# yugabyte/yugabyte-db

Measured on NVIDIA H100. Metric: compaction GB/s (input bytes merged), higher is better.
Workload: dtype u8

## Files before the change

yugabyte-db_b200/csrc/encode_kernels.cuh:

```cuda
#pragma once

namespace ybgpu {

constexpr int SEG = 4096;
constexpr int GROUP_SEGS = 64;

struct EncView {
  const RunView* runs;
  const Desc* kept;
  const ValueRewrite* rewrites;
  uint32_t* nr;
  uint16_t* shared;
  int16_t* D;
  unsigned long long* P;
  unsigned long long* QQ;
  uint32_t* next;
  uint32_t* exit1;
  uint32_t n;
  uint32_t ri;
  uint32_t ri_shift;
  uint32_t block_size;
  uint32_t deviation;
  uint32_t guess;
  int key_encoding;
// ... 130 lines not shown
  for (uint32_t base = 0; base < n; base += 1024) {
    uint32_t i = base + threadIdx.x;
    unsigned long long v = i < n ? a[i] : 0, x = v;
    for (int o = 1; o < 32; o <<= 1) { unsigned long long y = __shfl_up_sync(0xffffffffu, x, o); if (lane >= o) x += y; }
    if (lane == 31) ws[wid] = x;
    __syncthreads();
    if (wid == 0) {
      unsigned long long w = ws[lane];
      for (int o = 1; o < 32; o <<= 1) { unsigned long long y = __shfl_up_sync(0xffffffffu, w, o); if (lane >= o) w += y; }
      ws[lane] = w;
    }
    __syncthreads();
    if (i < n) a[i] = carry + (wid ? ws[wid - 1] : 0) + x - v;
    __syncthreads();
    if (threadIdx.x == 1023) carry += ws[31];
    __syncthreads();
  }
  if (threadIdx.x == 0 && total) *total = carry;
}
__global__ void __launch_bounds__(256) k_u64_chunk_sums(const unsigned long long* a, uint32_t n, unsigned long long* partial) {
  __shared__ unsigned long long sh;
  if (threadIdx.x == 0) sh = 0;
  __syncthreads();
  unsigned long long s = 0;
  const uint64_t base = static_cast<uint64_t>(blockIdx.x) * SCAN_CHUNK;
  for (uint32_t j = threadIdx.x; j < SCAN_CHUNK; j += 256) { const uint64_t i = base + j; if (i < n) s += a[i]; }
  for (int o = 16; o; o >>= 1) s += __shfl_xor_sync(0xffffffffu, s, o);
  if ((threadIdx.x & 31) == 0) atomicAdd(&sh, s);
  __syncthreads();
  if (threadIdx.x == 0) partial[blockIdx.x] = sh;
}
__global__ void __launch_bounds__(256) k_u64_chunk_final(unsigned long long* a, uint32_t n, const unsigned long long* partial) {
  __shared__ unsigned long long ws[8];
  const uint64_t base = static_cast<uint64_t>(blockIdx.x) * SCAN_CHUNK;
  constexpr int PER = SCAN_CHUNK / 256;
  const int lane = threadIdx.x & 31, wid = threadIdx.x >> 5;
  unsigned long long v[PER], s = 0;
  for (int j = 0; j < PER; j++) { const uint64_t i = base + threadIdx.x * PER + j; v[j] = i < n ? a[i] : 0; s += v[j]; }
  unsigned long long x = s;
  for (int o = 1; o < 32; o <<= 1) { const unsigned long long y = __shfl_up_sync(0xffffffffu, x, o); if (lane >= o) x += y; }
  if (lane == 31) ws[wid] = x;
  __syncthreads();
  unsigned long long run = partial[blockIdx.x] + x - s;
  for (int w = 0; w < wid; w++) run += ws[w];
  for (int j = 0; j < PER; j++) {
    const uint64_t i = base + threadIdx.x * PER + j;
    if (i < n) a[i] = run;
    run += v[j];
  }
}
__global__ void __launch_bounds__(256) k_p_final(const uint32_t* nr, uint32_t n, const unsigned long long* partial, unsigned long long* P) {
  __shared__ uint32_t warp_sums[32];
  const uint64_t base = static_cast<uint64_t>(blockIdx.x) * SCAN_CHUNK;
  constexpr int PER = SCAN_CHUNK / 256;
  uint32_t v[PER], s = 0;
  for (int j = 0; j < PER; j++) { uint64_t i = base + threadIdx.x * PER + j; v[j] = i < n ? nr[i] : 0; s += v[j]; }
  uint32_t off = block_exclusive_scan(s, warp_sums, nullptr);
  unsigned long long run = partial[blockIdx.x] + off;
  for (int j = 0; j < PER; j++) {
    uint64_t i = base + threadIdx.x * PER + j;
    if (i < n) P[i] = run;
    run += v[j];
    if (i + 1 == n) P[n] = run;
  }
}

constexpr int QROWS = 128;
__global__ void __launch_bounds__(256) k_qq_sums(const int16_t* D, uint32_t n, uint32_t ri, unsigned long long* partial , uint32_t nchunks) {
  const uint32_t t = blockIdx.x * blockDim.x + threadIdx.x;
  const uint32_t chunk = t / ri, col = t % ri;
  if (chunk >= nchunks) return;
  unsigned long long s = 0;
  for (int r = 0; r < QROWS; r++) {
    uint64_t i = (static_cast<uint64_t>(chunk) * QROWS + r) * ri + col;
    if (i < n) s += static_cast<unsigned long long>(static_cast<long long>(D[i]));
  }
  partial[static_cast<size_t>(col) * nchunks + chunk] = s;
}
__global__ void __launch_bounds__(256) k_qq_final(const int16_t* D, uint32_t n, uint32_t ri, const unsigned long long* partial, uint32_t nchunks, unsigned long long* QQ) {
  const uint32_t t = blockIdx.x * blockDim.x + threadIdx.x;
  const uint32_t chunk = t / ri, col = t % ri;
  if (chunk >= nchunks) return;
  unsigned long long s = partial[static_cast<size_t>(col) * nchunks + chunk];
  for (int r = 0; r < QROWS; r++) {
    uint64_t i = (static_cast<uint64_t>(chunk) * QROWS + r) * ri + col;
    if (i < n) { s += static_cast<unsigned long long>(static_cast<long long>(D[i])); QQ[i] = s; }
  }
}

__device__ __forceinline__ unsigned long long blk_cur(const EncView& E, uint32_t s, uint32_t j) {
  const uint32_t t = (j - s) >> E.ri_shift;
  return (E.P[j + 1] - E.P[s]) + (E.QQ[s + (t << E.ri_shift)] - E.QQ[s] + static_cast<unsigned long long>(static_cast<long long>(E.D[s]))) + 4ull * (t + 1) + 4ull;
}

__global__ void __launch_bounds__(256) k_next(EncView E) {
  const unsigned long long BS = E.block_size;
  const unsigned long long thresh = BS * (100 - E.deviation);
  const unsigned long long madd = *E.max_add;
  for (uint32_t s = blockIdx.x * blockDim.x + threadIdx.x; s < E.n; s += gridDim.x * blockDim.x) {
    uint32_t lo = s + 1, hi = E.n;
    if (E.deviation == 0) {
      while (lo < hi) { uint32_t mid = lo + ((hi - lo) >> 1); if (blk_cur(E, s, mid - 1) >= BS) hi = mid; else lo = mid + 1; }
      E.next[s] = lo;
      continue;
    }
    {
      uint32_t m = s + E.guess + (E.guess >> 3);
      for (int it = 0; it < 3 && lo < hi; it++) {
        if (m < lo) m = lo;
        if (m > hi) m = hi;
        const unsigned long long cur = blk_cur(E, s, m - 1);
        const unsigned long long have = cur * 100;
        const unsigned long long bpe = cur / (m - s) + 1;
        if (have > thresh) {
          hi = m;
          const unsigned long long over = (have - thresh) / 100;
          const unsigned long long back = over / bpe + 1;
          m = back >= m - s ? s + 1 : m - static_cast<uint32_t>(back);
        } else {
          lo = m < E.n ? m + 1 : E.n;
          const unsigned long long miss = (thresh - have) / 100;
          const unsigned long long fwd = miss / bpe + 1;
          m = fwd >= E.n - m ? E.n : m + static_cast<uint32_t>(fwd);
        }
      }
    }
    while (lo < hi) {
      uint32_t mid = lo + ((hi - lo) >> 1);
      if (blk_cur(E, s, mid - 1) * 100 > thresh) hi = mid; else lo = mid + 1;
    }
    uint32_t m = lo;
    if (m < E.n && BS > madd) {
      const unsigned long long lim = BS - madd;
      uint32_t a = m, b = E.n, g = m;
      for (int it = 0; it < 3 && a < b; it++) {
        if (g < a) g = a;
        if (g > b) g = b;
        const unsigned long long c = blk_cur(E, s, g - 1);
        const unsigned long long bpe = c / (g - s) + 1;
        if (c > lim) {
          b = g;
          const unsigned long long back = (c - lim) / bpe + 1;
          g = back >= g - a ? a : g - static_cast<uint32_t>(back);
        } else {
          a = g < E.n ? g + 1 : E.n;
          const unsigned long long fwd = (lim - c) / bpe + 1;
          g = fwd >= E.n - g ? E.n : g + static_cast<uint32_t>(fwd);
        }
      }
      while (a < b) {
        const uint32_t mid = a + ((b - a) >> 1);
        if (blk_cur(E, s, mid - 1) > lim) b = mid; else a = mid + 1;
      }
      m = a;
    }
    while (m < E.n) {
      const unsigned long long cur = blk_cur(E, s, m - 1);
      if (cur >= BS) break;
      const Desc d = E.kept[m];
      const unsigned long long est = cur + d.klen + d.vlen_out + ((((m - s) & (E.ri - 1)) == 0) ? 4 : 0) + 4 +
                                     varint_len(d.klen) + varint_len(d.vlen_out);
      if (est > BS && cur * 100 > thresh) break;
      m++;
    }
    E.next[s] = m;
  }
}

__global__ void __launch_bounds__(256) k_seg_exit(EncView E) {
  __shared__ uint32_t ex[SEG];
  const uint64_t b = static_cast<uint64_t>(blockIdx.x) * SEG;
  if (b >= E.n) return;
  const uint32_t e = static_cast<uint32_t>(umin64(b + SEG, E.n));
  const uint32_t cnt = e - static_cast<uint32_t>(b);
  for (uint32_t i = threadIdx.x; i < cnt; i += blockDim.x) ex[i] = E.next[b + i];
  __syncthreads();
  for (;;) {
    int changed = 0;
    for (uint32_t i = threadIdx.x; i < cnt; i += blockDim.x) {
      const uint32_t v = reinterpret_cast<volatile uint32_t*>(ex)[i];
      if (v < e) { reinterpret_cast<volatile uint32_t*>(ex)[i] = reinterpret_cast<volatile uint32_t*>(ex)[v - static_cast<uint32_t>(b)]; changed = 1; }
    }
    if (!__syncthreads_or(changed)) break;
  }
  for (uint32_t i = threadIdx.x; i < cnt; i += blockDim.x) E.exit1[b + i] = ex[i];
}

__global__ void __launch_bounds__(256) k_group_exit(EncView E, uint32_t* gexit, uint32_t ngroups) {
  const uint64_t t = blockIdx.x * static_cast<uint64_t>(blockDim.x) + threadIdx.x;
  const uint32_t g = static_cast<uint32_t>(t / SEG), q = static_cast<uint32_t>(t % SEG);
  if (g >= ngroups) return;
  const uint64_t gb = static_cast<uint64_t>(g) * SEG * GROUP_SEGS;
  const uint64_t ge = umin64(gb + static_cast<uint64_t>(SEG) * GROUP_SEGS, E.n);
  uint64_t s = gb + q;
  if (s >= E.n) { gexit[t] = E.n; return; }
  while (s < ge) s = E.exit1[s];
  gexit[t] = static_cast<uint32_t>(s);
}

__global__ void k_chain_groups(EncView E, const uint32_t* gexit, uint32_t ngroups, uint32_t* group_first) {
  if (threadIdx.x || blockIdx.x) return;
  for (uint32_t g = 0; g < ngroups; g++) group_first[g] = 0xffffffffu;
  uint64_t s = 0;
  const uint64_t GS = static_cast<uint64_t>(SEG) * GROUP_SEGS;
  while (s < E.n) {
    const uint32_t g = static_cast<uint32_t>(s / GS);
    if (group_first[g] == 0xffffffffu) group_first[g] = static_cast<uint32_t>(s);
    const uint64_t q = s - g * GS;
    if (q < SEG) s = gexit[static_cast<uint64_t>(g) * SEG + q];
    else s = E.exit1[s];
  }
}

__global__ void __launch_bounds__(128) k_group_fill(EncView E, const uint32_t* group_first, uint32_t ngroups, uint32_t* seg_first, uint32_t nsegs) {
  const uint32_t g = blockIdx.x * blockDim.x + threadIdx.x;
  if (g >= ngroups) return;
  const uint32_t s0 = static_cast<uint32_t>(g) * GROUP_SEGS, s1 = min(s0 + GROUP_SEGS, nsegs);
  for (uint32_t q = s0; q < s1; q++) seg_first[q] = 0xffffffffu;
  uint64_t s = group_first[g];
  if (s == 0xffffffffu) return;
  const uint64_t ge = umin64((static_cast<uint64_t>(g) + 1) * SEG * GROUP_SEGS, E.n);
  while (s < ge) {
    const uint32_t seg = static_cast<uint32_t>(s / SEG);
    if (seg_first[seg] == 0xffffffffu) seg_first[seg] = static_cast<uint32_t>(s);
    s = E.exit1[s];
  }
}

__global__ void __launch_bounds__(128) k_mark_starts(EncView E, const uint32_t* seg_first, uint32_t nsegs, uint8_t* is_start) {
  const uint32_t seg = blockIdx.x * blockDim.x + threadIdx.x;
  if (seg >= nsegs) return;
  uint64_t s = seg_first[seg];
  if (s == 0xffffffffu) return;
  const uint64_t e = umin64((static_cast<uint64_t>(seg) + 1) * SEG, E.n);
  while (s < e) { is_start[s] = 1; s = E.next[s]; }
}

__global__ void __launch_bounds__(256) k_start_sums(const uint8_t* is_start, uint32_t n, uint32_t* partial) {
  __shared__ uint32_t sh;
  if (threadIdx.x == 0) sh = 0;
  __syncthreads();
  uint32_t s = 0;
  const uint64_t base = static_cast<uint64_t>(blockIdx.x) * SCAN_CHUNK;
  for (uint32_t j = threadIdx.x; j < SCAN_CHUNK; j += 256) { uint64_t i = base + j; if (i < n) s += is_start[i]; }
  for (int o = 16; o; o >>= 1) s += __shfl_xor_sync(0xffffffffu, s, o);
  if ((threadIdx.x & 31) == 0) atomicAdd(&sh, s);
  __syncthreads();
  if (threadIdx.x == 0) partial[blockIdx.x] = sh;
}
__global__ void __launch_bounds__(256) k_block_first(const uint8_t* is_start, uint32_t n, const uint32_t* partial, uint32_t* block_first) {
  __shared__ uint32_t warp_sums[32];
  const uint64_t base = static_cast<uint64_t>(blockIdx.x) * SCAN_CHUNK;
  constexpr int PER = SCAN_CHUNK / 256;
  uint32_t s = 0;
  uint8_t f[PER];
  for (int j = 0; j < PER; j++) { uint64_t i = base + threadIdx.x * PER + j; f[j] = i < n ? is_start[i] : 0; s += f[j]; }
  uint32_t off = partial[blockIdx.x] + block_exclusive_scan(s, warp_sums, nullptr);
  for (int j = 0; j < PER; j++) if (f[j]) block_first[off++] = static_cast<uint32_t>(base + threadIdx.x * PER + j);
}

__global__ void __launch_bounds__(256) k_block_sizes(EncView E, const uint32_t* block_first, uint32_t nblocks, unsigned long long* block_off,
                                                     unsigned long long* max_size) {
  unsigned long long mx = 0;
  for (uint32_t b = blockIdx.x * blockDim.x + threadIdx.x; b < nblocks; b += gridDim.x * blockDim.x) {
    const uint32_t s = block_first[b], e = (b + 1 < nblocks) ? block_first[b + 1] : E.n;
    const unsigned long long sz = blk_cur(E, s, e - 1) + 5;
    block_off[b] = sz;
    mx = sz > mx ? sz : mx;
  }
  for (int o = 16; o; o >>= 1) { const unsigned long long y = __shfl_xor_sync(0xffffffffu, mx, o); mx = y > mx ? y : mx; }
  if ((threadIdx.x & 31) == 0 && mx) atomicMax(max_size, mx);
}

__device__ __forceinline__ int put_varint(uint8_t* p, uint32_t v) {
  int n = 0;
  while (v >= 128) { p[n++] = static_cast<uint8_t>(v | 128); v >>= 7; }
  p[n++] = static_cast<uint8_t>(v);
  return n;
}

__device__ uint32_t g_crc_tab[4][256];
__device__ uint32_t g_crc_x2n[32];
constexpr uint32_t CRC_XPOW_TABLE = 1u << 16;
__device__ uint32_t g_crc_xpow8[CRC_XPOW_TABLE + 1];
constexpr uint32_t CRC_STRIDE_WORDS = 256;
__device__ uint32_t g_crc_stride[4][256];
__device__ uint32_t g_crc_s32[4][256];

__global__ void k_crc_init() {
  const uint32_t i = threadIdx.x;
  uint32_t c = i;
  for (int k = 0; k < 8; k++) c = (c >> 1) ^ ((c & 1) ? 0x82F63B78u : 0u);
  g_crc_tab[0][i] = c;
  __syncthreads();
  for (int t = 1; t < 4; t++) {
    uint32_t prev = g_crc_tab[t - 1][i];
    g_crc_tab[t][i] = (prev >> 8) ^ g_crc_tab[0][prev & 0xff];
    __syncthreads();
  }
  if (i == 0) {
    auto mul = [](uint32_t a, uint32_t b) {
      uint32_t m = 1u << 31, p = 0;
      for (;;) {
        if (a & m) { p ^= b; if ((a & (m - 1)) == 0) break; }
        m >>= 1;
        b = (b & 1) ? (b >> 1) ^ 0x82F63B78u : b >> 1;
      }
      return p;
    };
// ... 1196 lines not shown
```

yugabyte-db_b200/csrc/engine.cu:

```cuda
#include "engine.h"
#include "host_sst.h"

#include <cuda_runtime.h>
#include <algorithm>
#include <cstdio>
#include <cstring>
#include <chrono>
#include <cstdlib>
#include <mutex>

namespace ybgpu {

#define CUDA_TRY(expr)                                                                      \
  do {                                                                                      \
    cudaError_t _e = (expr);                                                                \
    if (_e != cudaSuccess) {                                                                \
      return Fail(YBGPU_RUNTIME_ERROR, std::string(#expr) + ": " + cudaGetErrorString(_e)); \
    }                                                                                       \
  } while (0)

struct RunView {
  const uint8_t* data;
  const uint64_t* blk_off;
  const uint32_t* blk_size;
// ... 1271 lines not shown
    case DEV_ERR_BAD_ENTRY: return "bad entry in block";
    case DEV_ERR_COMPRESSED: return "compressed block (only kNoCompression, kSnappyCompression, kLZ4Compression and kLZ4HCCompression inputs are supported)";
    case DEV_ERR_KEY_TOO_LONG: return "key longer than the engine limit";
    case DEV_ERR_IRREGULAR_RESTARTS: return "data block restart intervals are not uniform";
    case DEV_ERR_BAD_KEY: return "cannot decode DocKey/SubDocKey components";
    case DEV_ERR_UNSUPPORTED_KEY: return "key component type not supported on the GPU path";
    case DEV_ERR_TILE_OVERFLOW: return "internal error: merge tile larger than its capacity";
    case DEV_ERR_BAD_HT: return "bad DocHybridTime at the end of a key";
    case DEV_ERR_BAD_VALUE: return "cannot decode value control fields";
    case DEV_ERR_STACK_DEPTH: return "too many subkey levels";
    case DEV_ERR_UNSUPPORTED_VALUE: return "record type needs a host callback (packed row / merge / single delete)";
    case DEV_ERR_BAD_CRC: return "block checksum mismatch";
    case DEV_ERR_COTABLE: return "cotable/colocated keys are not supported yet";
    case DEV_ERR_SHORT_KEY: return "internal key shorter than 8 bytes";
    case DEV_ERR_UNSORTED: return "input file is not sorted";
    default: return "unknown device error";
  }
}

static ybgpu_status DevErrorStatus(int e) {
  switch (e) {
    case DEV_ERR_COMPRESSED: case DEV_ERR_UNSUPPORTED_KEY: case DEV_ERR_UNSUPPORTED_VALUE:
    case DEV_ERR_TILE_OVERFLOW: case DEV_ERR_COTABLE: case DEV_ERR_KEY_TOO_LONG: case DEV_ERR_STACK_DEPTH:
    case DEV_ERR_IRREGULAR_RESTARTS:
      return YBGPU_NOT_SUPPORTED;
    default: return YBGPU_CORRUPTION;
  }
}

struct Engine::Impl {
  cudaStream_t stream = nullptr;
  bool owns_stream = false;
  uint8_t* status_host = nullptr; uint8_t* status_dev = nullptr;
  uint32_t readback_launches = 0;
  struct KvInput { const uint8_t* keys; const unsigned long long* koff; const unsigned long long* voff; uint32_t n; uint32_t max_klen; std::string last_user_key; };
  std::vector<KvInput> kv;
  std::vector<std::vector<uint32_t>> cf_oids;
  std::vector<std::vector<uint64_t>> cf_hts;
  uint8_t* staging_host = nullptr; uint8_t* staging_dev = nullptr;
  size_t upload_off = 0;
  cudaEvent_t ev0 = nullptr, ev1 = nullptr;
  cudaEvent_t phase_ev[8] = {};
  cudaEvent_t enc_ev[2] = {};
  bool enc_timed = false;
  cudaEvent_t snap_ev[4] = {};
  bool snap_timed = false;
  std::vector<void*> allocs;
  JobDev* dJ = nullptr;
  JobParams* dP = nullptr;
  RunView* dRuns = nullptr;
  std::vector<RunView> runs;
  std::vector<bool> owns_data;
  std::vector<std::vector<uint64_t>> keep_off; std::vector<std::vector<uint32_t>> keep_sz;
  uint8_t* out_keys = nullptr; uint64_t* out_koff = nullptr;
  uint8_t* out_vals = nullptr; uint64_t* out_voff = nullptr;
  uint64_t n_out = 0, out_key_bytes = 0, out_val_bytes = 0;
  JobDev hJ{};
  Desc* d_desc = nullptr; Sums3* d_partial = nullptr; ValueRewrite* d_rw = nullptr;
  uint64_t N = 0; int S = 0; uint32_t n_chunks = 0;
  bool kv_emitted = false;
  Desc* d_kept = nullptr;
  uint8_t* out_file = nullptr; uint64_t out_file_len = 0;
  uint32_t n_blocks = 0; unsigned long long* d_block_off = nullptr; uint32_t* d_block_first = nullptr;
  uint8_t* d_boundary = nullptr; uint32_t boundary_stride = 0;
  EncView enc{};
  cudaStream_t copy_stream = nullptr; cudaEvent_t copy_ev = nullptr; bool copy_pending = false;
  uint32_t n_filter_blocks = 0, filter_block_bytes = 0, filter_key_stride = 0;
  uint8_t* d_filters = nullptr; uint8_t* d_filter_keys = nullptr; uint32_t* d_filter_first = nullptr;
  BvOut* d_bv = nullptr;
};

__global__ void __launch_bounds__(256) k_records_from_kv(const uint8_t* keys, const unsigned long long* koff, const unsigned long long* voff,
                                                         const uint8_t* vals, uint32_t n, int S, uint8_t* rec, uint64_t* val_off, JobDev* J) {
  for (uint32_t i = blockIdx.x * blockDim.x + threadIdx.x; i < n; i += gridDim.x * blockDim.x) {
    const unsigned long long k0 = koff[i], k1 = koff[i + 1], v0 = voff[i], v1 = voff[i + 1];
    uint8_t* r = rec + static_cast<size_t>(i) * S;
    if (k1 < k0 + 8 || k1 - k0 - 8 > static_cast<unsigned long long>(S - 16) || v1 < v0 || v1 - v0 >= (1ull << 32)) {
      dev_fail(J, k1 < k0 + 8 ? DEV_ERR_SHORT_KEY : DEV_ERR_BAD_ENTRY, i);
      for (int b = 0; b < S; b++) r[b] = 0;
      val_off[i] = 0;
      continue;
    }
    const uint32_t ulen = static_cast<uint32_t>(k1 - k0 - 8), vlen = static_cast<uint32_t>(v1 - v0);
    const uint8_t* kp = keys + k0;
    for (int b = 0; b < S - 16; b++) r[b] = static_cast<uint32_t>(b) < ulen ? kp[b] : 0;
    uint64_t suffix = 0;
    for (int b = 7; b >= 0; b--) suffix = (suffix << 8) | kp[ulen + b];
    uint4 tr;
    tr.x = static_cast<uint32_t>(suffix); tr.y = static_cast<uint32_t>(suffix >> 32);
    tr.z = ulen | (static_cast<uint32_t>(vlen ? vals[v0] : 0) << 16);
    tr.w = vlen;
    *reinterpret_cast<uint4*>(r + S - 16) = tr;
    val_off[i] = v0;
  }
}

__global__ void k_readback(uint8_t* dst_mapped, const uint8_t* src, uint32_t n) {
  for (uint32_t i = threadIdx.x; i < n; i += blockDim.x) dst_mapped[i] = src[i];
  __threadfence_system();
}
constexpr size_t STATUS_READ_BYTES = 4096;
constexpr size_t STATUS_PAGE_BYTES = 65536;
struct StatusPage { uint8_t* host = nullptr; uint8_t* dev = nullptr; };
static std::mutex g_status_mu;
static std::vector<StatusPage> g_status_free;
static cudaError_t AcquireStatusPage(StatusPage* p) {
// ... 29 lines not shown
  if (e != cudaSuccess) { cudaFreeHost(h); return e; }
  p->host = static_cast<uint8_t*>(h); p->dev = static_cast<uint8_t*>(d);
  return cudaSuccess;
}
static void ReleaseStaging(const Staging& p) {
  if (!p.host) return;
  std::lock_guard<std::mutex> lock(g_status_mu);
  g_staging_free.push_back(p);
}
__global__ void __launch_bounds__(256) k_copy_out(uint8_t* dst_mapped, const uint8_t* src, size_t row_bytes, size_t src_pitch, size_t rows) {
  const size_t total = row_bytes * rows;
  const size_t stride = static_cast<size_t>(gridDim.x) * blockDim.x;
  if (src_pitch == row_bytes && ((reinterpret_cast<uintptr_t>(src) | reinterpret_cast<uintptr_t>(dst_mapped)) & 15) == 0) {
    const size_t nv = total >> 4;
    for (size_t i = blockIdx.x * static_cast<size_t>(blockDim.x) + threadIdx.x; i < nv; i += stride)
      reinterpret_cast<uint4*>(dst_mapped)[i] = reinterpret_cast<const uint4*>(src)[i];
    for (size_t i = (nv << 4) + blockIdx.x * static_cast<size_t>(blockDim.x) + threadIdx.x; i < total; i += stride) dst_mapped[i] = src[i];
  } else {
    for (size_t r = blockIdx.x; r < rows; r += gridDim.x)
      for (size_t c = threadIdx.x; c < row_bytes; c += blockDim.x) dst_mapped[r * row_bytes + c] = src[r * src_pitch + c];
  }
  __threadfence_system();
}

static bool ZeroCopyStatusEnabled() {
  const char* e = getenv("YBGPU_ZC_STATUS");
  return e ? atoi(e) != 0 : true;
}

Engine::Engine(const ybgpu_job_options& o) : opt_(o), impl_(new Impl) {
  if (o.largest_user_key && o.has_largest_user_key) largest_.assign(o.largest_user_key, o.largest_user_key + o.largest_user_key_len);
  if (o.key_bounds_lower_len) lower_.assign(o.key_bounds_lower, o.key_bounds_lower + o.key_bounds_lower_len);
  if (o.key_bounds_upper_len) upper_.assign(o.key_bounds_upper, o.key_bounds_upper + o.key_bounds_upper_len);
  if (o.range_lower_len) range_lower_.assign(o.range_lower, o.range_lower + o.range_lower_len);
  if (o.range_upper_len) range_upper_.assign(o.range_upper, o.range_upper + o.range_upper_len);
  opt_.range_lower = nullptr; opt_.range_upper = nullptr;
  opt_.largest_user_key = nullptr; opt_.key_bounds_lower = nullptr; opt_.key_bounds_upper = nullptr;
  memset(&stats_, 0, sizeof(stats_));
}

Engine::~Engine() {
  if (impl_) {
    cudaSetDevice(opt_.device);
    if (impl_->copy_pending) cudaStreamSynchronize(impl_->copy_stream);
    if (!ran_ && !impl_->runs.empty()) cudaStreamSynchronize(impl_->stream);
    for (void* p : impl_->allocs) cudaFreeAsync(p, impl_->stream);
    if (impl_->ev0) cudaEventDestroy(impl_->ev0);
    if (impl_->ev1) cudaEventDestroy(impl_->ev1);
    if (impl_->copy_stream) cudaStreamDestroy(impl_->copy_stream);
    if (impl_->copy_ev) cudaEventDestroy(impl_->copy_ev);
    for (auto& e : impl_->enc_ev) if (e) cudaEventDestroy(e);
    for (auto& e : impl_->snap_ev) if (e) cudaEventDestroy(e);
    for (auto& e : impl_->phase_ev) if (e) cudaEventDestroy(e);
    if (impl_->staging_host) { Staging st; st.host = impl_->staging_host; st.dev = impl_->staging_dev; ReleaseStaging(st); }
    if (impl_->status_host) {
      cudaStreamSynchronize(impl_->stream);
      StatusPage pg; pg.host = impl_->status_host; pg.dev = impl_->status_dev;
      ReleaseStatusPage(pg);
    }
    if (impl_->owns_stream && impl_->stream) cudaStreamDestroy(impl_->stream);
    delete impl_;
  }
}

ybgpu_status Engine::Fail(ybgpu_status s, const std::string& msg) { error_ = msg; return s; }

static thread_local cudaStream_t g_alloc_stream = nullptr;
template <typename T>
static cudaError_t DevAlloc(std::vector<void*>* allocs, T** out, size_t count) {
  void* p = nullptr;
  cudaError_t e = cudaMallocAsync(&p, std::max<size_t>(count * sizeof(T), 16) + 32, g_alloc_stream);
  if (e == cudaSuccess) { allocs->push_back(p); *out = reinterpret_cast<T*>(p); }
  return e;
}


static size_t CopyChunkBytes() {
  const char* e = getenv("YBGPU_COPY_CHUNK_MB");
  const long mb = e ? atol(e) : 32;
  return mb > 0 ? static_cast<size_t>(mb) << 20 : ~static_cast<size_t>(0);
}
static cudaError_t ChunkedCopyAsync(void* dst, const void* src, size_t len, cudaMemcpyKind kind, cudaStream_t stream) {
  const size_t chunk = CopyChunkBytes();
  for (size_t off = 0; off < len; off += chunk) {
    cudaError_t e = cudaMemcpyAsync(static_cast<uint8_t*>(dst) + off, static_cast<const uint8_t*>(src) + off, std::min(chunk, len - off), kind, stream);
    if (e != cudaSuccess) return e;
  }
  return cudaSuccess;
}

ybgpu_status Engine::Init() {
  int ndev = 0;
  cudaError_t e = cudaGetDeviceCount(&ndev);
  if (e != cudaSuccess || ndev == 0)
    return Fail(YBGPU_RUNTIME_ERROR, std::string("no usable CUDA device: ") + cudaGetErrorString(e) +
                                         " (this engine has no CPU fallback)");
  if (opt_.device < 0 || opt_.device >= ndev) return Fail(YBGPU_INVALID_ARGUMENT, "bad device ordinal");
  CUDA_TRY(cudaSetDevice(opt_.device));
  if (opt_.cuda_stream == YBGPU_STREAM_PRIVATE) {
    CUDA_TRY(cudaStreamCreateWithFlags(&impl_->stream, cudaStreamNonBlocking));
    impl_->owns_stream = true;
  } else {
    impl_->stream = reinterpret_cast<cudaStream_t>(opt_.cuda_stream);
  }
  g_alloc_stream = impl_->stream;
  {
    cudaMemPool_t pool;
    CUDA_TRY(cudaDeviceGetDefaultMemPool(&pool, opt_.device));
    uint64_t thr = ~0ull;
    CUDA_TRY(cudaMemPoolSetAttribute(pool, cudaMemPoolAttrReleaseThreshold, &thr));
    int off = 0;
    CUDA_TRY(cudaMemPoolSetAttribute(pool, cudaMemPoolReuseAllowInternalDependencies, &off));
  }
  if (ZeroCopyStatusEnabled()) {
    StatusPage pg;
    CUDA_TRY(AcquireStatusPage(&pg));
    impl_->status_host = pg.host; impl_->status_dev = pg.dev;
  }
  CUDA_TRY(cudaEventCreate(&impl_->ev0));
  CUDA_TRY(cudaEventCreate(&impl_->ev1));
  for (auto& e : impl_->phase_ev) CUDA_TRY(cudaEventCreate(&e));
  for (auto& e : impl_->enc_ev) CUDA_TRY(cudaEventCreate(&e));
  CUDA_TRY(DevAlloc(&impl_->allocs, &impl_->dJ, 1));
  CUDA_TRY(DevAlloc(&impl_->allocs, &impl_->dP, 1));
  CUDA_TRY(DevAlloc(&impl_->allocs, &impl_->dRuns, MAX_RUNS));
  return YBGPU_OK;
}

ybgpu_status Engine::AddInput(const uint8_t* data, uint64_t len, const ybgpu_block_handle* handles, uint64_t nh,
                              int key_encoding, uint64_t ht_filter, bool on_device) {
  if (ran_) return Fail(YBGPU_ILLEGAL_STATE, "add_input after run");
  if (impl_->runs.size() >= MAX_RUNS) return Fail(YBGPU_NOT_SUPPORTED, "too many input files");
  if (!impl_->kv.empty()) return Fail(YBGPU_NOT_SUPPORTED, "KV-stream inputs and table-file inputs cannot be mixed in one job");
  if (key_encoding != YBGPU_KEY_ENCODING_SHARED_PREFIX && key_encoding != YBGPU_KEY_ENCODING_THREE_SHARED_PARTS)
    return Fail(YBGPU_INVALID_ARGUMENT, "unknown data block key encoding");
  if (nh >= (1ull << 32)) return Fail(YBGPU_NOT_SUPPORTED, "too many data blocks in one file");
  CUDA_TRY(cudaSetDevice(opt_.device));
  g_alloc_stream = impl_->stream;
  for (uint64_t i = 0; i < nh; i++) {
    if (handles[i].offset > len || handles[i].size > len - handles[i].offset || len - handles[i].offset - handles[i].size < 5)
      return Fail(YBGPU_CORRUPTION, "block handle outside the data file");
    if (handles[i].size >= (1ull << 31)) return Fail(YBGPU_NOT_SUPPORTED, "data block too large");
  }
  RunView rv{};
  if (on_device) {
    rv.data = data;
  } else {
    uint8_t* d = nullptr;
    CUDA_TRY(DevAlloc(&impl_->allocs, &d, len + 64));
    CUDA_TRY(cudaMemsetAsync(d, 0, 16, impl_->stream));
    CUDA_TRY(ChunkedCopyAsync(d + 16, data, len, cudaMemcpyHostToDevice, impl_->stream));
    CUDA_TRY(cudaMemsetAsync(d + 16 + len, 0, 16, impl_->stream));
    rv.data = d + 16;
    stats_.h2d_bytes += len;
  }
  impl_->keep_off.emplace_back(nh); impl_->keep_sz.emplace_back(nh);
  std::vector<uint64_t>& off = impl_->keep_off.back(); std::vector<uint32_t>& sz = impl_->keep_sz.back();
  for (uint64_t i = 0; i < nh; i++) { off[i] = handles[i].offset; sz[i] = static_cast<uint32_t>(handles[i].size); }
  uint64_t* doff = nullptr; uint32_t* dsz = nullptr; uint32_t* dcnt = nullptr;
  CUDA_TRY(DevAlloc(&impl_->allocs, &doff, nh)); CUDA_TRY(DevAlloc(&impl_->allocs, &dsz, nh));
  CUDA_TRY(DevAlloc(&impl_->allocs, &dcnt, nh + 1));
  CUDA_TRY(cudaMemcpyAsync(doff, off.data(), nh * 8, cudaMemcpyHostToDevice, impl_->stream));
  CUDA_TRY(cudaMemcpyAsync(dsz, sz.data(), nh * 4, cudaMemcpyHostToDevice, impl_->stream));
  rv.blk_off = doff; rv.blk_size = dsz; rv.blk_count = dcnt; rv.nb = static_cast<uint32_t>(nh);
  rv.ht_filter = ht_filter;
  rv.key_encoding = static_cast<uint32_t>(key_encoding);
  impl_->runs.push_back(rv);
  impl_->cf_oids.emplace_back(); impl_->cf_hts.emplace_back();
  return YBGPU_OK;
}

ybgpu_status Engine::SetCotableFilters(const uint32_t* db_oids, const uint64_t* hybrid_times, uint32_t n) {
  if (ran_) return Fail(YBGPU_ILLEGAL_STATE, "set_cotable_filters after run");
  if (impl_->runs.empty()) return Fail(YBGPU_ILLEGAL_STATE, "set_cotable_filters before any input");
  if (n && (!db_oids || !hybrid_times)) return Fail(YBGPU_INVALID_ARGUMENT, "null cotable filter arrays");
  for (uint32_t i = 1; i < n; i++)
    if (db_oids[i - 1] >= db_oids[i]) return Fail(YBGPU_INVALID_ARGUMENT, "cotable filter database oids must be strictly increasing");
  impl_->cf_oids.back().assign(db_oids, db_oids + n);
  impl_->cf_hts.back().assign(hybrid_times, hybrid_times + n);
  return YBGPU_OK;
}

ybgpu_status Engine::AddInputKv(const uint8_t* keys, const uint64_t* key_offsets, const uint8_t* values, const uint64_t* value_offsets, uint64_t n) {
  Impl& I = *impl_;
  if (ran_) return Fail(YBGPU_ILLEGAL_STATE, "add_input after run");
  if (I.runs.size() >= MAX_RUNS) return Fail(YBGPU_NOT_SUPPORTED, "too many input files");
  if (I.kv.size() != I.runs.size()) return Fail(YBGPU_NOT_SUPPORTED, "KV-stream inputs and table-file inputs cannot be mixed in one job");
  if (n >= (1ull << 32)) return Fail(YBGPU_NOT_SUPPORTED, "more than 2^32 entries in one input");
  if (n && (!keys || !key_offsets || !value_offsets)) return Fail(YBGPU_INVALID_ARGUMENT, "null argument");
  CUDA_TRY(cudaSetDevice(opt_.device));
  g_alloc_stream = I.stream;
  const uint64_t kbytes = n ? key_offsets[n] : 0, vbytes = n ? value_offsets[n] : 0;
  uint32_t max_klen = 0;
  for (uint64_t i = 0; i < n; i++) {
    if (key_offsets[i + 1] < key_offsets[i] + 8 || value_offsets[i + 1] < value_offsets[i]) return Fail(YBGPU_INVALID_ARGUMENT, "bad key / value offsets");
    max_klen = std::max<uint32_t>(max_klen, static_cast<uint32_t>(std::min<uint64_t>(key_offsets[i + 1] - key_offsets[i], 0xffffffffu)));
  }
  uint8_t* dk = nullptr; uint8_t* dv = nullptr; unsigned long long* dko = nullptr; unsigned long long* dvo = nullptr; uint32_t* dcnt = nullptr;
  CUDA_TRY(DevAlloc(&I.allocs, &dk, kbytes + 16));
  CUDA_TRY(DevAlloc(&I.allocs, &dv, vbytes + 64));
  CUDA_TRY(DevAlloc(&I.allocs, &dko, n + 1)); CUDA_TRY(DevAlloc(&I.allocs, &dvo, n + 1)); CUDA_TRY(DevAlloc(&I.allocs, &dcnt, 1));
  CUDA_TRY(cudaMemsetAsync(dv, 0, 16, I.stream));
  if (kbytes) CUDA_TRY(ChunkedCopyAsync(dk, keys, kbytes, cudaMemcpyHostToDevice, I.stream));
  if (vbytes) CUDA_TRY(ChunkedCopyAsync(dv + 16, values, vbytes, cudaMemcpyHostToDevice, I.stream));
  CUDA_TRY(cudaMemsetAsync(dv + 16 + vbytes, 0, 16, I.stream));
  static const uint64_t zero_off[1] = {0};
  CUDA_TRY(ChunkedCopyAsync(dko, n ? key_offsets : zero_off, (n + 1) * 8, cudaMemcpyHostToDevice, I.stream));
  CUDA_TRY(ChunkedCopyAsync(dvo, n ? value_offsets : zero_off, (n + 1) * 8, cudaMemcpyHostToDevice, I.stream));
  stats_.h2d_bytes += kbytes + vbytes + 16 * (n + 1);
  RunView rv{};
  rv.data = dv + 16; rv.blk_off = nullptr; rv.blk_size = nullptr; rv.blk_count = dcnt; rv.nb = 0;
  rv.ht_filter = HT_FILTER_NONE; rv.key_encoding = YBGPU_KEY_ENCODING_SHARED_PREFIX;
  I.runs.push_back(rv);
  I.cf_oids.emplace_back(); I.cf_hts.emplace_back();
  Impl::KvInput ki{dk, dko, dvo, static_cast<uint32_t>(n), max_klen, std::string()};
  if (n) ki.last_user_key.assign(reinterpret_cast<const char*>(keys + key_offsets[n - 1]), key_offsets[n] - key_offsets[n - 1] - 8);
// ... 521 lines not shown
  launches += 2;
  I.d_desc = d_desc; I.d_partial = d_partial; I.d_rw = d_rw; I.N = N; I.S = Sfinal; I.n_chunks = n_chunks;
  if (I.n_out >= (1ull << 32)) return Fail(YBGPU_NOT_SUPPORTED, "too many output entries");
  const uint32_t n = static_cast<uint32_t>(I.n_out);
  if (n) {
    const uint32_t ri = static_cast<uint32_t>(opt_.block_restart_interval);
    if (ri == 0 || (ri & (ri - 1)) || ri > 64)
      return Fail(YBGPU_NOT_SUPPORTED, "block_restart_interval must be a power of two <= 64 for the GPU block encoder");
    if (opt_.output_key_encoding != YBGPU_KEY_ENCODING_SHARED_PREFIX && opt_.output_key_encoding != YBGPU_KEY_ENCODING_THREE_SHARED_PARTS)
      return Fail(YBGPU_INVALID_ARGUMENT, "unknown output_key_encoding");
    if (static_cast<uint64_t>(n) == N) {
      I.d_kept = d_desc;
    } else {
      CUDA_TRY(DevAlloc(&I.allocs, &I.d_kept, n));
      k_compact_desc<<<n_chunks, EMIT_THREADS, 0, I.stream>>>(d_desc, N, d_partial, I.d_kept);
    }
    EncView& E = I.enc;
    E.runs = I.dRuns; E.kept = I.d_kept; E.rewrites = d_rw; E.n = n; E.ri = ri;
    E.ri_shift = 0; while ((1u << E.ri_shift) < ri) E.ri_shift++;
    E.key_encoding = opt_.output_key_encoding;
    E.block_size = opt_.block_size; E.deviation = static_cast<uint32_t>(std::max(0, opt_.block_size_deviation));
    {
      const double avg = static_cast<double>(I.out_key_bytes + I.out_val_bytes) / n + 3.0;
      E.guess = static_cast<uint32_t>(std::max(1.0, 0.85 * opt_.block_size / avg));
    }
    CUDA_TRY(DevAlloc(&I.allocs, &E.nr, n)); CUDA_TRY(DevAlloc(&I.allocs, &E.shared, n)); CUDA_TRY(DevAlloc(&I.allocs, &E.D, n));
    CUDA_TRY(DevAlloc(&I.allocs, &E.P, static_cast<size_t>(n) + 1)); CUDA_TRY(DevAlloc(&I.allocs, &E.QQ, n));
    CUDA_TRY(DevAlloc(&I.allocs, &E.next, n)); CUDA_TRY(DevAlloc(&I.allocs, &E.exit1, n));
    E.fk_len = nullptr; E.fk_src = nullptr; E.fkh_src = nullptr;
    if (opt_.filter_policy != YBGPU_FILTER_NONE) {
      if (opt_.filter_policy != YBGPU_FILTER_DOCKEY_V3) return Fail(YBGPU_INVALID_ARGUMENT, "unknown filter_policy");
      CUDA_TRY(DevAlloc(&I.allocs, &E.fk_len, n));
      E.fk_src = d_fk16;
      E.fkh_src = d_fkh;
    }
    CUDA_TRY(DevAlloc(&I.allocs, &E.max_add, 1));
    CUDA_TRY(cudaMemsetAsync(E.max_add, 0, 4, I.stream));
    k_entry_sizes<<<GridFor(n, 256, sms), 256, 0, I.stream>>>(E, Sfinal);
    const uint32_t pc = (n + SCAN_CHUNK - 1) / SCAN_CHUNK;
    unsigned long long* d_pp = nullptr;
    CUDA_TRY(DevAlloc(&I.allocs, &d_pp, pc + 1));
    k_p_sums<<<pc, 256, 0, I.stream>>>(E.nr, n, d_pp);
    k_scan_u64_single<<<1, 1024, 0, I.stream>>>(d_pp, pc, nullptr);
    k_p_final<<<pc, 256, 0, I.stream>>>(E.nr, n, d_pp, E.P);
    const uint32_t rows = (n + ri - 1) / ri;
    const uint32_t qchunks = (rows + QROWS - 1) / QROWS;
    unsigned long long* d_qp = nullptr;
    CUDA_TRY(DevAlloc(&I.allocs, &d_qp, static_cast<size_t>(qchunks) * ri + 1));
    const uint32_t qthreads = qchunks * ri;
    k_qq_sums<<<(qthreads + 255) / 256, 256, 0, I.stream>>>(E.D, n, ri, d_qp, qchunks);
    k_scan_u64_single<<<ri, 1024, 0, I.stream>>>(d_qp, qchunks, nullptr, qchunks);
    k_qq_final<<<(qthreads + 255) / 256, 256, 0, I.stream>>>(E.D, n, ri, d_qp, qchunks, E.QQ);
    launches += 8;
    k_next<<<GridFor(n, 256, sms), 256, 0, I.stream>>>(E);
    const uint32_t nsegs = (n + SEG - 1) / SEG;
    const uint32_t ngroups = (nsegs + GROUP_SEGS - 1) / GROUP_SEGS;
    uint32_t *d_gexit = nullptr, *d_group_first = nullptr, *d_seg_first = nullptr, *d_spart = nullptr, *d_nblocks = nullptr;
    uint8_t* d_is_start = nullptr;
    CUDA_TRY(DevAlloc(&I.allocs, &d_gexit, static_cast<size_t>(ngroups) * SEG));
    CUDA_TRY(DevAlloc(&I.allocs, &d_group_first, ngroups)); CUDA_TRY(DevAlloc(&I.allocs, &d_seg_first, nsegs));
    CUDA_TRY(DevAlloc(&I.allocs, &d_is_start, n)); CUDA_TRY(DevAlloc(&I.allocs, &d_spart, pc + 1)); CUDA_TRY(DevAlloc(&I.allocs, &d_nblocks, 1));
    CUDA_TRY(cudaMemsetAsync(d_is_start, 0, n, I.stream));
    k_seg_exit<<<nsegs, 256, 0, I.stream>>>(E);
    k_group_exit<<<static_cast<uint32_t>((static_cast<uint64_t>(ngroups) * SEG + 255) / 256), 256, 0, I.stream>>>(E, d_gexit, ngroups);
    k_chain_groups<<<1, 32, 0, I.stream>>>(E, d_gexit, ngroups, d_group_first);
    k_group_fill<<<(ngroups + 127) / 128, 128, 0, I.stream>>>(E, d_group_first, ngroups, d_seg_first, nsegs);
    k_mark_starts<<<(nsegs + 127) / 128, 128, 0, I.stream>>>(E, d_seg_first, nsegs, d_is_start);
    k_start_sums<<<pc, 256, 0, I.stream>>>(d_is_start, n, d_spart);
    k_scan_u32_single<<<1, 1024, 0, I.stream>>>(d_spart, pc, d_nblocks);
    launches += 8;
    uint32_t nblocks = 0;
    if (ybgpu_status s = ReadSmall(&nblocks, d_nblocks, 4)) return s;
    I.n_blocks = nblocks;
    CUDA_TRY(DevAlloc(&I.allocs, &I.d_block_first, static_cast<size_t>(nblocks) + 1));
    CUDA_TRY(DevAlloc(&I.allocs, &I.d_block_off, static_cast<size_t>(nblocks) + 1));
    unsigned long long* d_total = nullptr;
    CUDA_TRY(DevAlloc(&I.allocs, &d_total, 2));
    CUDA_TRY(cudaMemsetAsync(d_total, 0, 16, I.stream));
    k_block_first<<<pc, 256, 0, I.stream>>>(d_is_start, n, d_spart, I.d_block_first);
    k_block_sizes<<<GridFor(nblocks, 256, sms), 256, 0, I.stream>>>(E, I.d_block_first, nblocks, I.d_block_off, d_total + 1);
    {
      const uint32_t bc = (nblocks + SCAN_CHUNK - 1) / SCAN_CHUNK;
      unsigned long long* d_bpart = nullptr;
      CUDA_TRY(DevAlloc(&I.allocs, &d_bpart, static_cast<size_t>(bc) + 1));
      k_u64_chunk_sums<<<bc, 256, 0, I.stream>>>(I.d_block_off, nblocks, d_bpart);
      k_scan_u64_single<<<1, 1024, 0, I.stream>>>(d_bpart, bc, d_total);
      k_u64_chunk_final<<<bc, 256, 0, I.stream>>>(I.d_block_off, nblocks, d_bpart);
      launches += 2;
    }
    unsigned long long total_and_max[2] = {0, 0};
    if (ybgpu_status s = ReadSmall(total_and_max, d_total, 16)) return s;
    const unsigned long long total = total_and_max[0];
    if (ybgpu_status us = UploadSmall(I.d_block_off + nblocks, &total, 8)) return us;
    I.out_file_len = total;
    CUDA_TRY(DevAlloc(&I.allocs, &I.out_file, total + 64));
    {
      const size_t esm = ENC_SMEM_CAP + 32;
      const bool tsp = E.key_encoding == YBGPU_KEY_ENCODING_THREE_SHARED_PARTS;
      const bool v3 = getenv("YBGPU_ENC_V3") != nullptr;
      const uint32_t G = ((4u + 28u + static_cast<uint32_t>(Sfinal) + 32u + 7u) & ~7u) + 4u;
      const size_t v5_smem = 4096 + static_cast<size_t>(ENC5_THREADS) * G;
      const bool v5 = !v3 && getenv("YBGPU_ENC_V4") == nullptr && v5_smem <= 96 * 1024;
      if (!v3) stats_.path_flags |= YBGPU_PATH_ENCODER_V4;
      CUDA_TRY(cudaEventRecord(I.enc_ev[0], I.stream));
      if (v5) {
        stats_.path_flags |= YBGPU_PATH_ENCODER_V5;
        auto kern = tsp ? k_encode_v5<2> : k_encode_v5<1>;
// ... 356 lines not shown
```

Measured before the change: 258.5.

## Warm-start block boundary search, coalesce P scan, vectorize start loads, pin handle staging

k_next now gives each warp a run of consecutive start entries and seeds every boundary search from the previous answer, using exponential galloping instead of a fixed guess plus bisection, so fewer blk_cur evaluations are needed. k_p_final switches to a strided, coalesced per-iteration block scan. The start-marker scan reads 16 bytes per thread with a single vector load. Block handles are staged in pinned host memory so the H2D copies are truly asynchronous, and the staging buffer is released only after the stream syncs. A profiling script is also added.

```diff
diff --git a/profiles/step_kernels.py b/profiles/step_kernels.py
--- /dev/null
+++ b/profiles/step_kernels.py
@@ -0,0 +1,146 @@
+import argparse
+import collections
+import importlib
+import json
+import os
+import re
+import subprocess
+import sys
+import tempfile
+import time
+
+ROOT = os.path.dirname(os.path.dirname(os.path.abspath(__file__)))
+sys.path[:0] = [ROOT]
+
+
+def short_name(name):
+    name = re.sub(r"^void ", "", name)
+    name = name.split("(")[0]
+    name = re.sub(r"<.*", "", name)
+    return name.split("::")[-1]
+
+
+def phase_of_sequence(names):
+    labels, phase = [], "ingest+decode"
+    for nm in names:
+        if phase == "ingest+decode" and nm == "k_sample_pos":
+            phase = "partition"
+        elif phase == "partition" and nm == "k_merge_filter":
+            phase = "merge"
+        elif phase == "merge" and nm != "k_merge_filter":
+            phase = "encode"
+        if phase == "encode" and nm.startswith("k_encode"):
+            labels.append("assembler")
+        else:
+            labels.append(phase)
+    return labels
+
+
+def main():
+    ap = argparse.ArgumentParser()
+    ap.add_argument("--rows", type=int, default=None, help="entries in the job (default: bench.py's headline shape)")
+    ap.add_argument("--jobs", type=int, default=3, help="jobs per measurement")
+    ap.add_argument("--warmup", type=int, default=2)
+    args = ap.parse_args()
+
+    import torch
+    from torch.profiler import ProfilerActivity, profile
+    import bench
+    pkg = importlib.import_module("yugabyte-db_b200")
+    if not torch.cuda.is_available() or pkg.device_count() < 1:
+        raise SystemExit("step_kernels.py needs a CUDA device")
+    smi = subprocess.run(["nvidia-smi", "--query-gpu=name,power.limit,clocks.max.sm", "--format=csv,noheader", "-i", "0"],
+                         capture_output=True, text=True).stdout.strip()
+    print("card: %s" % smi)
+
+    rows = args.rows or bench.DEFAULT_ROWS
+    cfg = pkg.GenConfig(seed=2, num_rows=rows, cols=1, versions=1, num_files=bench.NUM_FILES, value_len=bench.VALUE_LEN,
+                        row_offset=0, hash_rows_total=rows)
+    ssts = pkg.generate_ssts(cfg, max_threads=bench.NUM_FILES)
+    handles = [bench.read_handles(pkg, s) for s in ssts]
+    dev = []
+    for s in ssts:
+        v = s.data_view()
+        t = torch.empty(v.size + 64, dtype=torch.uint8, device="cuda")
+        t[16:16 + v.size].copy_(torch.from_numpy(v))
+        dev.append(t)
+    stream_ptr = torch.cuda.current_stream().cuda_stream
+    torch.cuda.synchronize()
+
+    def job_once():
+        job = pkg.GpuCompactionJob(device=0, verify_checksums=True, cuda_stream=stream_ptr, filter_policy=1)
+        t0 = time.perf_counter()
+        for t, s, (off, sz) in zip(dev, ssts, handles):
+            job.add_input_device(t.data_ptr() + 16, s.data_view().size, off, sz)
+        t1 = time.perf_counter()
+        st = job.run().as_dict()
+        t2 = time.perf_counter()
+        job.close()
+        return (t1 - t0) * 1e3, (t2 - t1) * 1e3, st
+
+    for _ in range(args.warmup):
+        job_once()
+    torch.cuda.synchronize()
+    host = [job_once() for _ in range(args.jobs)]
+    torch.cuda.synchronize()
+    add_ms = sorted(h[0] for h in host)
+    run_ms = sorted(h[1] for h in host)
+    st = host[-1][2]
+    print("host ms per job: add_input_device x%d files %s (median %.3f), run %s (median %.3f)" % (
+        len(ssts), ["%.3f" % x for x in add_ms], add_ms[len(add_ms) // 2], ["%.2f" % x for x in run_ms], run_ms[len(run_ms) // 2]))
+    print("engine phase ms (CUDA events, last job; slot 5 = block assembler): %s; gpu_kernel_launches %d" % (
+        ["%.3f" % (x * 1e3) for x in st["phase_seconds"][:6]], st["gpu_kernel_launches"]))
+
+    with tempfile.TemporaryDirectory() as td:
+        with profile(activities=[ProfilerActivity.CUDA]) as prof:
+            for _ in range(args.jobs):
+                job_once()
+            torch.cuda.synchronize()
+        path = os.path.join(td, "trace.json")
+        prof.export_chrome_trace(path)
+        with open(path) as f:
+            trace = json.load(f)
+    ops = [e for e in trace.get("traceEvents", []) if e.get("ph") == "X" and e.get("cat") in ("kernel", "gpu_memset", "gpu_memcpy")]
+    ops.sort(key=lambda e: e["ts"])
+    names = [short_name(e["name"]) if e["cat"] == "kernel" else e["cat"] for e in ops]
+    jobs, cur = [], []
+    for e, nm in zip(ops, names):
+        cur.append((e, nm))
+        if nm == "k_boundary_keys":
+            jobs.append(cur)
+            cur = []
+    if cur:
+        jobs[-1:] = [jobs[-1] + cur] if jobs else [cur]
+    nj = len(jobs)
+    print("profiled jobs: %d (device operations %d)" % (nj, len(ops)))
+    per_kernel = collections.OrderedDict()
+    per_phase = collections.OrderedDict()
+    for job in jobs:
+        labels = phase_of_sequence([nm for _, nm in job])
+        prev_end, prev_label = None, None
+        for (e, nm), lab in zip(job, labels):
+            key = (lab, nm)
+            k = per_kernel.setdefault(key, [0.0, 0])
+            k[0] += e["dur"]
+            k[1] += 1
+            p = per_phase.setdefault(lab, {"busy": 0.0, "gap": 0.0, "launches": 0, "first": e["ts"], "last": 0.0})
+            p["busy"] += e["dur"]
+            p["launches"] += 1 if e["cat"] == "kernel" else 0
+            if prev_end is not None and prev_label == lab:
+                p["gap"] += max(0.0, e["ts"] - prev_end)
+            prev_end, prev_label = e["ts"] + e["dur"], lab
+    print("\n%-16s %-28s %10s %8s" % ("phase", "operation", "ms/job", "n/job"))
+    for (lab, nm), (us, cnt) in per_kernel.items():
+        print("%-16s %-28s %10.3f %8.1f" % (lab, nm, us / 1e3 / nj, cnt / nj))
+    print("\n%-16s %10s %10s %10s" % ("phase", "busy ms", "gaps ms", "launches"))
+    tot = [0.0, 0.0, 0]
+    for lab, p in per_phase.items():
+        print("%-16s %10.3f %10.3f %10.1f" % (lab, p["busy"] / 1e3 / nj, p["gap"] / 1e3 / nj, p["launches"] / nj))
+        tot[0] += p["busy"]; tot[1] += p["gap"]; tot[2] += p["launches"]
+    print("%-16s %10.3f %10.3f %10.1f" % ("all", tot[0] / 1e3 / nj, tot[1] / 1e3 / nj, tot[2] / nj))
+    outside = sum(p["busy"] + p["gap"] for lab, p in per_phase.items() if lab in ("partition", "encode"))
+    print("partition + encode phase without the assembler (busy + gaps): %.3f ms/job" % (outside / 1e3 / nj))
+
+
+if __name__ == "__main__":
+    main()
diff --git a/yugabyte-db_b200/csrc/encode_kernels.cuh b/yugabyte-db_b200/csrc/encode_kernels.cuh
--- a/yugabyte-db_b200/csrc/encode_kernels.cuh
+++ b/yugabyte-db_b200/csrc/encode_kernels.cuh
@@ -206,16 +206,15 @@
 __global__ void __launch_bounds__(256) k_p_final(const uint32_t* nr, uint32_t n, const unsigned long long* partial, unsigned long long* P) {
   __shared__ uint32_t warp_sums[32];
   const uint64_t base = static_cast<uint64_t>(blockIdx.x) * SCAN_CHUNK;
-  constexpr int PER = SCAN_CHUNK / 256;
-  uint32_t v[PER], s = 0;
-  for (int j = 0; j < PER; j++) { uint64_t i = base + threadIdx.x * PER + j; v[j] = i < n ? nr[i] : 0; s += v[j]; }
-  uint32_t off = block_exclusive_scan(s, warp_sums, nullptr);
-  unsigned long long run = partial[blockIdx.x] + off;
-  for (int j = 0; j < PER; j++) {
-    uint64_t i = base + threadIdx.x * PER + j;
-    if (i < n) P[i] = run;
-    run += v[j];
-    if (i + 1 == n) P[n] = run;
+  unsigned long long run = partial[blockIdx.x];
+  for (uint32_t r = 0; r < SCAN_CHUNK; r += 256) {
+    const uint64_t i = base + r + threadIdx.x;
+    const uint32_t v = i < n ? nr[i] : 0;
+    uint32_t tot;
+    const uint32_t off = block_exclusive_scan(v, warp_sums, &tot);
+    if (i < n) P[i] = run + off;
+    if (i + 1 == n) P[n] = run + off + v;
+    run += tot;
   }
 }
 
@@ -247,77 +246,71 @@
   return (E.P[j + 1] - E.P[s]) + (E.QQ[s + (t << E.ri_shift)] - E.QQ[s] + static_cast<unsigned long long>(static_cast<long long>(E.D[s]))) + 4ull * (t + 1) + 4ull;
 }
 
+template <class Pred>
+__device__ __forceinline__ uint32_t first_true_from(uint32_t lo, uint32_t hi, uint32_t h, Pred pred) {
+  uint32_t a = lo, b = hi;
+  h = h < a ? a : h > b ? b : h;
+  if (h < b) {
+    if (pred(h)) {
+      b = h;
+      for (uint32_t st = 1; b > a; st <<= 1) {
+        const uint32_t x = b - a > st ? b - st : a;
+        if (pred(x)) b = x; else { a = x + 1; break; }
+      }
+    } else {
+      a = h + 1;
+      for (uint32_t st = 1; a < b; st <<= 1) {
+        const uint32_t x = b - a > st - 1 ? a + st - 1 : b;
+        if (x >= b) break;
+        if (pred(x)) { b = x; break; }
+        a = x + 1;
+      }
+    }
+  }
+  while (a < b) {
+    const uint32_t mid = a + ((b - a) >> 1);
+    if (pred(mid)) b = mid; else a = mid + 1;
+  }
+  return a;
+}
+
+constexpr uint32_t NEXT_RUN = 8;
+
 __global__ void __launch_bounds__(256) k_next(EncView E) {
   const unsigned long long BS = E.block_size;
   const unsigned long long thresh = BS * (100 - E.deviation);
   const unsigned long long madd = *E.max_add;
-  for (uint32_t s = blockIdx.x * blockDim.x + threadIdx.x; s < E.n; s += gridDim.x * blockDim.x) {
-    uint32_t lo = s + 1, hi = E.n;
-    if (E.deviation == 0) {
-      while (lo < hi) { uint32_t mid = lo + ((hi - lo) >> 1); if (blk_cur(E, s, mid - 1) >= BS) hi = mid; else lo = mid + 1; }
-      E.next[s] = lo;
-      continue;
-    }
-    {
-      uint32_t m = s + E.guess + (E.guess >> 3);
-      for (int it = 0; it < 3 && lo < hi; it++) {
-        if (m < lo) m = lo;
-        if (m > hi) m = hi;
+  const uint32_t lane = threadIdx.x & 31;
+  const uint32_t chunks = (E.n + 32 * NEXT_RUN - 1) / (32 * NEXT_RUN);
+  const uint32_t wpg = (gridDim.x * blockDim.x) >> 5;
+  for (uint32_t c = (blockIdx.x * blockDim.x + threadIdx.x) >> 5; c < chunks; c += wpg) {
+    const uint32_t s0 = c * 32 * NEXT_RUN + lane, s1 = min(c * 32 * NEXT_RUN + 32 * NEXT_RUN, E.n);
+    uint32_t hint1 = s0 + E.guess + (E.guess >> 3) - 32, hint2 = hint1;
+    for (uint32_t s = s0; s < s1; s += 32, hint1 += 32, hint2 += 32) {
+      uint32_t m;
+      if (E.deviation == 0) {
+        m = first_true_from(s + 1, E.n, hint1, [&](uint32_t x) { return blk_cur(E, s, x - 1) >= BS; });
+        E.next[s] = hint1 = m;
+        continue;
+      }
+      m = first_true_from(s + 1, E.n, hint1, [&](uint32_t x) { return blk_cur(E, s, x - 1) * 100 > thresh; });
+      hint1 = m;
+      if (m < E.n && BS > madd) {
+        const unsigned long long lim = BS - madd;
+        m = first_true_from(m, E.n, max(hint2, m), [&](uint32_t x) { return blk_cur(E, s, x - 1) > lim; });
+        hint2 = m;
+      }
+      while (m < E.n) {
         const unsigned long long cur = blk_cur(E, s, m - 1);
-        const unsigned long long have = cur * 100;
-        const unsigned long long bpe = cur / (m - s) + 1;
-        if (have > thresh) {
-          hi = m;
-          const unsigned long long over = (have - thresh) / 100;
-          const unsigned long long back = over / bpe + 1;
-          m = back >= m - s ? s + 1 : m - static_cast<uint32_t>(back);
-        } else {
-          lo = m < E.n ? m + 1 : E.n;
-          const unsigned long long miss = (thresh - have) / 100;
-          const unsigned long long fwd = miss / bpe + 1;
-          m = fwd >= E.n - m ? E.n : m + static_cast<uint32_t>(fwd);
-        }
-      }
-    }
-    while (lo < hi) {
-      uint32_t mid = lo + ((hi - lo) >> 1);
-      if (blk_cur(E, s, mid - 1) * 100 > thresh) hi = mid; else lo = mid + 1;
-    }
-    uint32_t m = lo;
-    if (m < E.n && BS > madd) {
-      const unsigned long long lim = BS - madd;
-      uint32_t a = m, b = E.n, g = m;
-      for (int it = 0; it < 3 && a < b; it++) {
-        if (g < a) g = a;
-        if (g > b) g = b;
-        const unsigned long long c = blk_cur(E, s, g - 1);
-        const unsigned long long bpe = c / (g - s) + 1;
-        if (c > lim) {
-          b = g;
-          const unsigned long long back = (c - lim) / bpe + 1;
-          g = back >= g - a ? a : g - static_cast<uint32_t>(back);
-        } else {
-          a = g < E.n ? g + 1 : E.n;
-          const unsigned long long fwd = (lim - c) / bpe + 1;
-          g = fwd >= E.n - g ? E.n : g + static_cast<uint32_t>(fwd);
-        }
-      }
-      while (a < b) {
-        const uint32_t mid = a + ((b - a) >> 1);
-        if (blk_cur(E, s, mid - 1) > lim) b = mid; else a = mid + 1;
-      }
-      m = a;
-    }
-    while (m < E.n) {
-      const unsigned long long cur = blk_cur(E, s, m - 1);
-      if (cur >= BS) break;
-      const Desc d = E.kept[m];
-      const unsigned long long est = cur + d.klen + d.vlen_out + ((((m - s) & (E.ri - 1)) == 0) ? 4 : 0) + 4 +
-                                     varint_len(d.klen) + varint_len(d.vlen_out);
-      if (est > BS && cur * 100 > thresh) break;
-      m++;
-    }
-    E.next[s] = m;
+        if (cur >= BS) break;
+        const Desc d = E.kept[m];
+        const unsigned long long est = cur + d.klen + d.vlen_out + ((((m - s) & (E.ri - 1)) == 0) ? 4 : 0) + 4 +
+                                       varint_len(d.klen) + varint_len(d.vlen_out);
+        if (est > BS && cur * 100 > thresh) break;
+        m++;
+      }
+      E.next[s] = m;
+    }
   }
 }
 
@@ -406,9 +399,18 @@
   __shared__ uint32_t warp_sums[32];
   const uint64_t base = static_cast<uint64_t>(blockIdx.x) * SCAN_CHUNK;
   constexpr int PER = SCAN_CHUNK / 256;
+  static_assert(PER == 16, "one 16-byte load per thread");
   uint32_t s = 0;
   uint8_t f[PER];
-  for (int j = 0; j < PER; j++) { uint64_t i = base + threadIdx.x * PER + j; f[j] = i < n ? is_start[i] : 0; s += f[j]; }
+  const uint64_t i0 = base + threadIdx.x * PER;
+  if (i0 + PER <= n && (reinterpret_cast<uintptr_t>(is_start) & 15) == 0) {
+    const uint4 w = *reinterpret_cast<const uint4*>(is_start + i0);
+    const uint32_t ws[4] = {w.x, w.y, w.z, w.w};
+    for (int j = 0; j < PER; j++) f[j] = static_cast<uint8_t>(ws[j >> 2] >> (8 * (j & 3)));
+  } else {
+    for (int j = 0; j < PER; j++) { const uint64_t i = i0 + j; f[j] = i < n ? is_start[i] : 0; }
+  }
+  for (int j = 0; j < PER; j++) s += f[j];
   uint32_t off = partial[blockIdx.x] + block_exclusive_scan(s, warp_sums, nullptr);
   for (int j = 0; j < PER; j++) if (f[j]) block_first[off++] = static_cast<uint32_t>(base + threadIdx.x * PER + j);
 }
diff --git a/yugabyte-db_b200/csrc/engine.cu b/yugabyte-db_b200/csrc/engine.cu
--- a/yugabyte-db_b200/csrc/engine.cu
+++ b/yugabyte-db_b200/csrc/engine.cu
@@ -1347,6 +1347,7 @@
   std::vector<RunView> runs;
   std::vector<bool> owns_data;
   std::vector<std::vector<uint64_t>> keep_off; std::vector<std::vector<uint32_t>> keep_sz;
+  size_t handles_staged = 0;
   uint8_t* out_keys = nullptr; uint64_t* out_koff = nullptr;
   uint8_t* out_vals = nullptr; uint64_t* out_voff = nullptr;
   uint64_t n_out = 0, out_key_bytes = 0, out_val_bytes = 0;
@@ -1482,7 +1483,10 @@
     for (auto& e : impl_->enc_ev) if (e) cudaEventDestroy(e);
     for (auto& e : impl_->snap_ev) if (e) cudaEventDestroy(e);
     for (auto& e : impl_->phase_ev) if (e) cudaEventDestroy(e);
-    if (impl_->staging_host) { Staging st; st.host = impl_->staging_host; st.dev = impl_->staging_dev; ReleaseStaging(st); }
+    if (impl_->staging_host) {
+      cudaStreamSynchronize(impl_->stream);
+      Staging st; st.host = impl_->staging_host; st.dev = impl_->staging_dev; ReleaseStaging(st);
+    }
     if (impl_->status_host) {
       cudaStreamSynchronize(impl_->stream);
       StatusPage pg; pg.host = impl_->status_host; pg.dev = impl_->status_dev;
@@ -1584,14 +1588,27 @@
     rv.data = d + 16;
     stats_.h2d_bytes += len;
   }
-  impl_->keep_off.emplace_back(nh); impl_->keep_sz.emplace_back(nh);
-  std::vector<uint64_t>& off = impl_->keep_off.back(); std::vector<uint32_t>& sz = impl_->keep_sz.back();
+  if (!impl_->staging_host) {
+    Staging st;
+    if (AcquireStaging(&st) == cudaSuccess) { impl_->staging_host = st.host; impl_->staging_dev = st.dev; }
+    else (void)cudaGetLastError();
+  }
+  const size_t off_bytes = (nh * 8 + 15) & ~static_cast<size_t>(15), sz_bytes = (nh * 4 + 15) & ~static_cast<size_t>(15);
+  uint64_t* off; uint32_t* sz;
+  if (impl_->staging_host && impl_->handles_staged + off_bytes + sz_bytes <= STAGING_BYTES) {
+    off = reinterpret_cast<uint64_t*>(impl_->staging_host + impl_->handles_staged);
+    sz = reinterpret_cast<uint32_t*>(impl_->staging_host + impl_->handles_staged + off_bytes);
+    impl_->handles_staged += off_bytes + sz_bytes;
+  } else {
+    impl_->keep_off.emplace_back(nh); impl_->keep_sz.emplace_back(nh);
+    off = impl_->keep_off.back().data(); sz = impl_->keep_sz.back().data();
+  }
   for (uint64_t i = 0; i < nh; i++) { off[i] = handles[i].offset; sz[i] = static_cast<uint32_t>(handles[i].size); }
   uint64_t* doff = nullptr; uint32_t* dsz = nullptr; uint32_t* dcnt = nullptr;
   CUDA_TRY(DevAlloc(&impl_->allocs, &doff, nh)); CUDA_TRY(DevAlloc(&impl_->allocs, &dsz, nh));
   CUDA_TRY(DevAlloc(&impl_->allocs, &dcnt, nh + 1));
-  CUDA_TRY(cudaMemcpyAsync(doff, off.data(), nh * 8, cudaMemcpyHostToDevice, impl_->stream));
-  CUDA_TRY(cudaMemcpyAsync(dsz, sz.data(), nh * 4, cudaMemcpyHostToDevice, impl_->stream));
+  CUDA_TRY(cudaMemcpyAsync(doff, off, nh * 8, cudaMemcpyHostToDevice, impl_->stream));
+  CUDA_TRY(cudaMemcpyAsync(dsz, sz, nh * 4, cudaMemcpyHostToDevice, impl_->stream));
   rv.blk_off = doff; rv.blk_size = dsz; rv.blk_count = dcnt; rv.nb = static_cast<uint32_t>(nh);
   rv.ht_filter = ht_filter;
   rv.key_encoding = static_cast<uint32_t>(key_encoding);
@@ -2219,7 +2236,7 @@
     k_scan_u64_single<<<ri, 1024, 0, I.stream>>>(d_qp, qchunks, nullptr, qchunks);
     k_qq_final<<<(qthreads + 255) / 256, 256, 0, I.stream>>>(E.D, n, ri, d_qp, qchunks, E.QQ);
     launches += 8;
-    k_next<<<GridFor(n, 256, sms), 256, 0, I.stream>>>(E);
+    k_next<<<GridFor((static_cast<uint64_t>(n) + NEXT_RUN - 1) / NEXT_RUN, 256, sms), 256, 0, I.stream>>>(E);
     const uint32_t nsegs = (n + SEG - 1) / SEG;
     const uint32_t ngroups = (nsegs + GROUP_SEGS - 1) / GROUP_SEGS;
     uint32_t *d_gexit = nullptr, *d_group_first = nullptr, *d_seg_first = nullptr, *d_spart = nullptr, *d_nblocks = nullptr;
```

Result: faster. 269.4, median of 6 (+4.2%).
